# jsh58/Genrich

Hardware: AMD Instinct MI355X
Metric: genome bases p-scored/sec, hg38 50M frags (higher is better)
Workload: dtype int32 pileup (1/120 units) + f64 p-values; 1 GPU; hg38 25 contigs (3088286401 bp), 50000000 paired fragments x 1 replicate(s), treatment only, -p 0.01 (BASELINE.json configs[1]); parallelism=chromosome-sharded x1, collectives=none, rccl_nranks=0, intervals=83948696, tables_written_in_step=none: the sweep walks the loose (end, V) slots, p = table p(V)

## Files before the change

### genrich_amd/csrc/gx_host_ctx.h

```cpp
#pragma once
#include <hip/hip_runtime.h>
#include <rocprim/device/device_radix_sort.hpp>

#include <algorithm>
#include <cmath>
#include <cstdio>
#include <cstdlib>
#include <cstring>
#include <atomic>
#include <chrono>
#include <string>
#include <vector>
#include <unistd.h>

#include "gx_merge.h"
#include "gx_rccl.h"
#include "gx_sort.h"
#include "gx_tile_fast.h"
#include "gx_sbtile.h"
#include "gx_dups.h"
#include "gx_bhx.h"
#include "gx_saturate.h"
#include "gx_count.h"
#include "gx_regions.h"
#include "gx_coverage.h"
#include "gx_profile.h"
#include "gx_gram.h"
#include "gx_fingerprint.h"
#include "gx_rank.h"

using namespace gx;

namespace {

struct DevBuf {
  void* p = nullptr;
  size_t cap = 0;
  DevBuf() = default;
  DevBuf(const DevBuf&) = delete;
  DevBuf& operator=(const DevBuf&) = delete;
  DevBuf(DevBuf&& o) noexcept : p(o.p), cap(o.cap), own(o.own) { o.p = nullptr; o.cap = 0; o.own = true; }
  DevBuf& operator=(DevBuf&& o) noexcept {
    if (this != &o) { release(); p = o.p; cap = o.cap; own = o.own; o.p = nullptr; o.cap = 0; o.own = true; }
    return *this;
  }
  ~DevBuf() { release(); }
  void release() {
    if (p && own) (void)hipFree(p);
    p = nullptr;
    cap = 0;
    own = true;
  }
  void view(void* ptr, size_t bytes) {
    release();
    p = ptr;
    cap = bytes;
    own = false;
  }
  hipError_t ensure(size_t bytes) {
    if (bytes <= cap) return hipSuccess;
    release();
    size_t want = bytes + bytes / 8 + 256;
    hipError_t e = hipMalloc(&p, want);
    if (e == hipSuccess) cap = want;
    return e;
  }
  template <typename T> T* as() const { return reinterpret_cast<T*>(p); }
  bool own = true;
};

struct HostMail {
  Scalars scal;
  long long acc[2];
  uint64_t peakBP, genome;
  u32 nF, nIv, status, R, nPeaks, nMerged, D, n, hot, bhOvf;
  long long coll[4];
  u32 counts[64];
  u32 closeState;
  u32 statusKeep;
  u32 seq;
};

struct PinnedBuf {
  void* p = nullptr;
  void* dp = nullptr;
  size_t cap = 0;
  PinnedBuf() = default;
  PinnedBuf(const PinnedBuf&) = delete;
  PinnedBuf& operator=(const PinnedBuf&) = delete;
  ~PinnedBuf() { if (p) (void)hipHostFree(p); }
  hipError_t ensure(size_t bytes) {
    if (bytes <= cap) return hipSuccess;
    if (p) (void)hipHostFree(p);
    p = nullptr;
    cap = 0;
    size_t want = bytes + bytes / 4 + 4096;
    hipError_t e = hipHostMalloc(&p, want, hipHostMallocMapped | hipHostMallocCoherent);
    if (e == hipSuccess) {
      cap = want;
      e = hipHostGetDevicePointer(&dp, p, 0);
    }
    return e;
  }
};

struct Pileup {
  DevBuf ivEnd, ivV, tileIvOff, chromIvOff;
  u32 nIv = 0;
  bool packed = false;
  DevBuf looseEnd, looseV, meta;
  bool inLoose = false;
};

struct PArray {
  DevBuf end, p, expt, ctrl, chromOff, tileOff, q, dPresent;
  u32 n = 0;
  bool loose = false;
  bool looseSweep = false;
  DevBuf chromLooseOff;
  size_t looseStride = 0;
  bool pilesPending = false;
  bool pairPending = false;
  bool mergedP = false;
  DevBuf keptV, keptMeta;
  bool keptLoose = false;
  bool latePending = false, lateLoose = false;
  bool qLazy = false;
  bool hasPiles = false;
  bool pilesDropped = false;
  float ctrlConst = 0.0f;
  bool ctrlIsConst = false;
  std::vector<uint8_t> present;
};

struct Phase {
  std::string name;
  hipEvent_t a, b;
};

struct Knobs {
  int debug = 0;
  int debugRetry = 0;
  int noSpin = 0;
  int forceRec64 = 0;
  int forceSlowFrag = 0;
  int noFused = 0;
  int noLoose = 0;
  int noPairs = 0;
  int noFracPairs = 0;
  int noBedFused = 0;
  int bhVariant = -1;
  int mergeWg = 0;
  int noQLoose = 0;
  int noLateLoose = 0;
  int noLazyQ = 0;
  int noPackHist = 0;
  int noMergeP = 0;
  int forceHalfBins = 0;
  int noHalfBins = 0;
  int fracHalfBins = 0;
  int noEarlyColl = 0;
  int regWindows = 0;
  int noDenseBh = 0;
  int qtMulti = 0;
  int forceColl = 0;
  int sbShift = -1;
  long long runCapMin = 0;
  int bhCapLog = 0;
  int ptJmax = 0;
  int sbtTr = 0;
  int sbtGrid = 0;
  int s2Grid = 0;
  int fpAgg = 0;
  int rankCapLog = 0;
  int rankLookup = 0;
  int roctx = 0;
  int fault = 0;
};
struct BuildPlan {
  int isCtrl = 0;
  bool reuseSort = false;
  u32 nEv = 0;
  bool unit32 = false;
  bool multiRank = false;
  bool earlyColl = false;
  bool fused = false;
  bool pairs = false;
  bool fracPairs = false;
  int sbS = 0;
  u32 nL1 = 0;
  u32 nCoarse = 0, jmaxC = 0, nWG1 = 0;
  u32 jmax = 0;
  u32 poolPages[3] = {0, 0, 0};
  bool wantEarly = false;
  bool wantLate = false;
  bool closeInScan = false;
  bool dense = false;
  bool denseSmall = false;
  bool fragFused = false;
  size_t looseCap = 0, ivCap = 0;
  u32 tChunks = 0;
  bool masks() const { return wantEarly || wantLate; }
};
struct KnobDef { const char* name; int Knobs::*i; long long Knobs::*ll; };
const KnobDef KNOBS[] = {
    {"GX_DEBUG", &Knobs::debug, nullptr}, {"GX_DEBUG_RETRY", &Knobs::debugRetry, nullptr}, {"GX_NO_SPIN", &Knobs::noSpin, nullptr},
    {"GX_FORCE_REC64", &Knobs::forceRec64, nullptr}, {"GX_FORCE_SLOWFRAG", &Knobs::forceSlowFrag, nullptr},
    {"GX_NO_FUSED", &Knobs::noFused, nullptr}, {"GX_NO_LOOSE", &Knobs::noLoose, nullptr}, {"GX_NO_PAIRS", &Knobs::noPairs, nullptr},
    {"GX_NO_FRAC_PAIRS", &Knobs::noFracPairs, nullptr}, {"GX_NO_BED_FUSED", &Knobs::noBedFused, nullptr}, {"GX_NO_MERGE_P", &Knobs::noMergeP, nullptr}, {"GX_NO_PACK_HIST", &Knobs::noPackHist, nullptr}, {"GX_NO_LAZY_Q", &Knobs::noLazyQ, nullptr}, {"GX_NO_LATE_LOOSE", &Knobs::noLateLoose, nullptr}, {"GX_NO_Q_LOOSE", &Knobs::noQLoose, nullptr}, {"GX_MERGE_WG", &Knobs::mergeWg, nullptr}, {"GX_BH_VARIANT", &Knobs::bhVariant, nullptr}, {"GX_FORCE_HALF_BINS", &Knobs::forceHalfBins, nullptr},
    {"GX_NO_HALF_BINS", &Knobs::noHalfBins, nullptr}, {"GX_FRAC_HALF_BINS", &Knobs::fracHalfBins, nullptr}, {"GX_NO_EARLY_COLL", &Knobs::noEarlyColl, nullptr},
    {"GX_NO_DENSE_BH", &Knobs::noDenseBh, nullptr}, {"GX_REG_WINDOWS", &Knobs::regWindows, nullptr}, {"GX_QT_MULTI", &Knobs::qtMulti, nullptr}, {"GX_FORCE_COLL", &Knobs::forceColl, nullptr},
    {"GX_SBSHIFT", &Knobs::sbShift, nullptr}, {"GX_RUN_CAP_MIN", nullptr, &Knobs::runCapMin}, {"GX_BH_CAPLOG", &Knobs::bhCapLog, nullptr},
    {"GX_PT_JMAX", &Knobs::ptJmax, nullptr}, {"GX_FAULT", &Knobs::fault, nullptr}, {"GX_SBT_TR", &Knobs::sbtTr, nullptr}, {"GX_SBT_GRID", &Knobs::sbtGrid, nullptr},
    {"GX_S2_GRID", &Knobs::s2Grid, nullptr},
    {"GX_FP_AGG", &Knobs::fpAgg, nullptr},
    {"GX_RANK_CAP_LOG", &Knobs::rankCapLog, nullptr},
    {"GX_RANK_LOOKUP", &Knobs::rankLookup, nullptr},
    {"GX_ROCTX", &Knobs::roctx, nullptr},
};
bool set_knob(Knobs& k, const char* name, const char* value) {
  for (const KnobDef& d : KNOBS)
    if (!strcmp(d.name, name)) {
      long long v = 1;
      if (value && *value) {
        char* end = nullptr;
        v = strtoll(value, &end, 10);
        if (end == value) v = 1;
      }
      if (d.i) k.*(d.i) = (int)v; else k.*(d.ll) = v;
      return true;
    }
  return false;
}

}

struct gx_ctx {
  gx_params par{};
  Knobs knob;
  int device = 0;
  hipStream_t stream = nullptr;
  bool keepPiles = true;
  int maskIdx = -1;
  u32 maskN = 0;
  size_t maskStride = 0;
  hipStream_t side = nullptr;
  hipEvent_t sideEv = nullptr;
  std::string err;
  std::vector<uint32_t> len;
  std::vector<uint8_t> skip, save, owned;
  std::vector<std::vector<uint32_t>> bed;
  std::vector<DChrom> hChrom;
  u32 nChrom = 0, nTiles = 0;
  int sbShift = 0;
  u32 nSB = 0;
  DevBuf dChrom, dTileChrom, dBedTileOff, dBedEdge, dTileSave0;
  bool hasBed = false;
  bool bedGiven = false;
  size_t nBedEdges = 0;
  int phase = 0;
  int sample = 0;
  struct Seg { const gx_event* p; size_t n; hipEvent_t ready; bool packed = false; };
  std::vector<DevBuf> unpackBufs;
  size_t unpackUsed = 0;
  std::vector<Seg> segs;
  std::vector<DevBuf> evChunks;
  size_t evChunkIdx = 0, evChunkFill = 0;
  PinnedBuf stage[2];
  hipEvent_t stageFree[2] = {nullptr, nullptr};
  int stageNext = 0;
  std::vector<hipEvent_t> evPool;
  size_t evPoolUsed = 0;
  DevBuf satBuf;
  struct Stream {
    DevBuf a, pool, pt, cursor, sbOff;
  };
  size_t b2LdsSet = 0;
  bool sbtLdsSet = false;
  bool sawFrac = false;
  bool fracHint = false;
  bool fusedOff = false;
  BuildPlan built;
  bool earlyOwed = false;
  bool earlyPending = false;
  int fusedBackoff[2] = {0, 0};
  bool looseSwept = false;
  bool pilesMade = false;
  int denseHistIdx = -1;
  bool denseHistUsed = false;
  bool mergePUsed = false;
  DevBuf lbSweep, lbSweep2;
  u32 sweepGen = 0;
  FragSelect closeSel{};
  u32 closeSeq = 0;
  bool beginPending = false;
  u64 beginGenome = 0;
  bool fellBack = false;
  bool ptGrew = false;
  bool packedUsed = false;
  bool looseOk = false;
  bool riskNearThr = false;
  size_t looseStride = 0;
  DevBuf tileSlot, chromW0, chromLooseOff, looseCtl;
  u32 ptJmax = 16;
  DevBuf lbIv;
  Stream str[3];
  DevBuf tileCnt[3], tileOff[3];
  DevBuf looseC, looseC2, pairLogE, pairCtab, pairP2d, fragSum, tileDeep, fragList, zeroArena, endAtLen, binNet, curC, ptC, poolC, auxC, nWide, wideList, heavyList;
  size_t arenaBytes = 0;
  DevBuf tileMeta, tileWsum, tileCarry, lb, misc, dScal, dStatus, looseEnd, looseV, tileIvCount, tileLastEnd, tilePrevEnd;
  Pileup expt, ctrl;
  Scalars hScal{};
  std::vector<PArray> reps;
  int finalIdx = -1;
  DevBuf pvLut, dRisk, dDeep;
  PinnedBuf riskHost;
  bool pairTabsReady = false;
  DevBuf bhKeys, bhLens, bhOutKeys, bhOutSlot, bhSortKeys, bhSortSlot, bhQ, bhKQ, bhRaw, bhDl, bhTmp, bhRecs;
  PinnedBuf hostRecs;
  bool satDone = false;
  long long satDropped = 0;
  bool qLooseBad = false;
  bool qLooseUsed = false;
  DevBuf qLut;
  bool lateLooseUsed = false;
  bool lazyQUsed = false;
  bool bhLive = false;
  u32 bhLiveCap = 0;
  int bhLiveIdx = -1;
  bool bhDirty = false;
  u32 bhCapLog = 22;
  DevBuf swStart, swEnd, swMask, cand, valid, peaks, headPos, candHdr, longList;
  PinnedBuf hPeaks;
  size_t nHostPeaks = 0;
  u32* nIvTarget = nullptr;
  PinnedBuf mailBuf;
  HostMail* mail = nullptr;
  uint64_t genomeLenUsed = 0, peakBP = 0;
  int rank = 0, world = 1;
  gx_allreduce_i64_fn allreduce = nullptr;
  void* user = nullptr;
  ncclComm_t comm = nullptr;
  bool forceColl = false;
  DevBuf bigBins;
  DevBuf dColl, dCounts, dGather, bhDense, bhxSmall, bhxRecv, bhxKeys, bhxLens, bhxQ, bhxOut, bhxAns;
  bool rangeBhUsed = false;
  bool denseBhUsed = false;
  int phaseLevel = 0;
  std::string phaseFilter = "tile";
  u32 mailSeq = 0;
  u32 statusSeen = 1;
  u64 runCap = 0, runSeen = 0;
  bool phaseOpen = false;
  bool roctxOpen = false;
  int numCU = 0, resTile = 0, resTileHalf = 0, resTileFast = 0, resSweep = 0;
  int resSortA = 0, resSortB = 0;
  std::vector<DevBuf> pool;
  struct KeptSample {
    int rep = 0;
    bool ctrl = false;
    std::vector<Seg> segs;
    std::vector<uint8_t> save;
    std::vector<DevBuf> chunks, unpacks;
    DevBuf sat;
  };
  bool countOn = false;
  bool peaksReady = false;
// ... 293 lines not shown
```

### genrich_amd/csrc/gx_host_sweep.h

```cpp
#pragma once
namespace {

struct SweepSrc {
  const u32* end = nullptr;
  const float* p = nullptr;
  const float* q = nullptr;
  const u64* kq = nullptr;
  u32 kqMask = 0;
  const int* V = nullptr;
  const float* qLut = nullptr;
  bool haveMasks = false, hasSkip = true;
  const u32* chromOff = nullptr;
  u32 nChrom = 0, nWords = 0;
  size_t mStride = 0;
};

int run_sweep(gx_ctx* ctx, const SweepSrc& S, u32* nPeaksOut) {
  hipStream_t s = ctx->stream;
  u32* misc = ctx->misc.as<u32>();
  HostMail* dm = static_cast<HostMail*>(ctx->mailBuf.dp);
  const u32 nWords = S.nWords, nChrom = S.nChrom;
  const u32 wChunks = (nWords + SW_CHUNK - 1) / SW_CHUNK;
  SweepMasks SM{ctx->swMask.as<u64>(), ctx->swMask.as<u64>() + S.mStride, ctx->swMask.as<u64>() + 2 * S.mStride, nWords};
  if (S.V) SM = SweepMasks{ctx->swMask.as<u64>(), nullptr, ctx->swMask.as<u64>() + S.mStride, nWords};
  u32 R = 0, nPeaks = 0;
  ctx->peakBP = 0;
  ctx->nHostPeaks = 0;
  if (nWords) {
    if (!S.V) hipLaunchKernelGGL(k_brk_mask, dim3((nChrom + 255) / 256), dim3(256), 0, s, S.chromOff, nChrom, SM.brk);
    if (!S.haveMasks)
      hipLaunchKernelGGL(k_sig_mask, dim3(std::max(1u, std::min((nWords + 15) / 16, 4096u))), dim3(256), 0, s, S.p, S.q,
                         misc + M_NIV, ctx->par.thr, SM);
    {
      const size_t need = (size_t)2 * (wChunks + 8) * 8;
      if (ctx->lbSweep.cap < need) {
        HIPCHECK(ctx->lbSweep.ensure(need));
        HIPCHECK(hipMemsetAsync(ctx->lbSweep.p, 0, ctx->lbSweep.cap, s));
      }
    }
    for (int attempt = 0;; attempt++) {
      const u64 capMin = ctx->knob.runCapMin > 0 ? (u64)ctx->knob.runCapMin : (u64)1 << 16;
      const u64 guess = ctx->knob.runCapMin > 0 ? capMin : std::max<u64>(capMin, (u64)nWords / 4);
      const u32 cap = std::min<u64>(std::max<u64>(ctx->runCap, std::max<u64>(guess, 1)), (u64)nWords * 64);
      HIPCHECK(ctx->swStart.ensure((size_t)cap * 4 + 16));
      HIPCHECK(ctx->swEnd.ensure((size_t)cap * 4 + 16));
      HIPCHECK(ctx->headPos.ensure((size_t)cap * 4 + 16));
      HIPCHECK(ctx->cand.ensure((size_t)cap * sizeof(gx_peak)));
      HIPCHECK(ctx->valid.ensure((size_t)cap * 4 + 16));
      HIPCHECK(ctx->hPeaks.ensure((size_t)cap * sizeof(gx_peak) + 16));
      HIPCHECK(ctx->candHdr.ensure((size_t)cap * sizeof(uint4)));
      HIPCHECK(ctx->longList.ensure((size_t)cap * 4 + 16));
      const u32 rChunks = (cap + RC_CHUNK - 1) / RC_CHUNK;
      {
        const size_t need = (size_t)2 * (rChunks + 8) * 8;
        if (ctx->lbSweep2.cap < need) {
          HIPCHECK(ctx->lbSweep2.ensure(need));
          HIPCHECK(hipMemsetAsync(ctx->lbSweep2.p, 0, ctx->lbSweep2.cap, s));
        }
      }
      if (++ctx->sweepGen >= (1u << 24)) {
        ctx->sweepGen = 1;
        HIPCHECK(hipMemsetAsync(ctx->lbSweep.p, 0, ctx->lbSweep.cap, s));
        HIPCHECK(hipMemsetAsync(ctx->lbSweep2.p, 0, ctx->lbSweep2.cap, s));
      }
      const u32 gen = ctx->sweepGen;
      u64* lbS = ctx->lbSweep.as<u64>();
      u64* lbE = lbS + wChunks + 8;
      u64* lbC = ctx->lbSweep2.as<u64>();
      u64* lbP = lbC + rChunks + 8;
      u32* runStart = ctx->swStart.as<u32>();
      u32* runEnd = ctx->swEnd.as<u32>();
      const u64* skipM = S.hasSkip ? SM.skip : (const u64*)nullptr;
      const u32 gridP = (u32)std::max(1, ctx->resSweep);
      hipLaunchKernelGGL(k_runs, dim3(std::min<u32>(wChunks, gridP)), dim3(SW_NT), 0, s, SM, lbS, lbE, gen, runStart, runEnd, cap,
                         misc + M_SWCOUNT, &dm->R, misc + M_TICKET3, reinterpret_cast<u64*>(misc + M_PEAKBP), ctx->dStatus.as<u32>());
      hipLaunchKernelGGL(k_cands, dim3(std::min<u32>(rChunks, gridP)), dim3(SW_NT), 0, s, SM, skipM, S.end, runStart, runEnd,
                         misc + M_SWCOUNT, ctx->par.max_gap, S.chromOff, nChrom, lbC, gen, ctx->headPos.as<u32>(), misc + M_NHEADS,
                         ctx->dStatus.as<u32>());
      hipLaunchKernelGGL(k_cand_hdr, dim3(std::max(1u, std::min((cap + 255) / 256, 4096u))), dim3(256), 0, s, SM, S.end, runStart,
                         runEnd, misc + M_SWCOUNT, ctx->headPos.as<u32>(), misc + M_NHEADS, ctx->candHdr.as<uint4>(),
                         ctx->longList.as<u32>(), misc + M_TICKET3);
      if (S.kq)
        hipLaunchKernelGGL(k_q_fill_cands, dim3(std::max(1u, std::min((cap + 3) / 4, 32768u))), dim3(256), 0, s,
                           ctx->candHdr.as<uint4>(), misc + M_NHEADS, S.p, S.kq, S.kqMask, const_cast<float*>(S.q), ctx->dStatus.as<u32>());
      {
        const dim3 grid(std::max(1u, std::min((cap + 15) / 16, 16384u)));
        const dim3 gridW(std::max(1u, std::min((cap + 3) / 4, (u32)(8 * ctx->numCU))));
#define GX_LAUNCH_PEAKS(Q, V, NSHORT, QPTR)                                                                               \
  hipLaunchKernelGGL((k_peak_both<Q, V>), dim3((NSHORT) + gridW.x), dim3(256), 0, s, (u32)(NSHORT), ctx->candHdr.as<uint4>(), \
                     S.end, S.p, QPTR, S.chromOff, nChrom, misc + M_NHEADS, ctx->longList.as<u32>(), misc + M_TICKET3,       \
                     ctx->par.thr, ctx->par.min_auc, ctx->par.min_len, ctx->cand.as<gx_peak>(), ctx->valid.as<u32>())
        if (S.V && S.qLut) {
          const u32 nShortV = std::min<u32>(grid.x, (u32)(8 * ctx->numCU));
          hipLaunchKernelGGL((k_peak_both<false, true, true>), dim3(nShortV + gridW.x), dim3(256), 0, s, nShortV, ctx->candHdr.as<uint4>(),
                             S.end, S.p, reinterpret_cast<const float*>(S.V), S.chromOff, nChrom, misc + M_NHEADS, ctx->longList.as<u32>(),
                             misc + M_TICKET3, ctx->par.thr, ctx->par.min_auc, ctx->par.min_len, ctx->cand.as<gx_peak>(),
                             ctx->valid.as<u32>(), S.qLut);
        } else if (S.V) {
          const u32 nShortV = std::min<u32>(grid.x, (u32)(8 * ctx->numCU));
          GX_LAUNCH_PEAKS(false, true, nShortV, reinterpret_cast<const float*>(S.V));
        } else if (S.q)
          GX_LAUNCH_PEAKS(true, false, grid.x, S.q);
        else
          GX_LAUNCH_PEAKS(false, false, grid.x, S.q);
#undef GX_LAUNCH_PEAKS
      }
      hipLaunchKernelGGL(k_peaks, dim3(std::min<u32>(rChunks, gridP)), dim3(SW_NT), 0, s, ctx->cand.as<gx_peak>(), ctx->valid.as<u32>(),
                         misc + M_NHEADS, lbP, gen, static_cast<gx_peak*>(ctx->hPeaks.dp), misc + M_NPEAKS, &dm->nPeaks,
                         ctx->dStatus.as<u32>(), reinterpret_cast<u64*>(misc + M_PEAKBP));
      if (int rc__ = dbg_sync(ctx, "sweep kernels")) return rc__;
      if (int rc__ = mail_sync(ctx, nullptr, nullptr, nullptr, nullptr, nullptr, reinterpret_cast<const u64*>(misc + M_PEAKBP)))
        return rc__;
      R = ctx->mail->R;
      ctx->runSeen = R;
      if (R <= cap) break;
      if (attempt >= 2) {
        ctx->err = "peak sweep: run count changed between attempts";
        return GX_ERR_DEVICE;
      }
      ctx->runCap = (u64)R + R / 4 + 1024;
    }
    ctx->runCap = std::max<u64>(ctx->runCap, (u64)R + R / 4 + 1024);
  } else {
    if (int rc__ = mail_sync(ctx, nullptr, nullptr, nullptr, nullptr, nullptr)) return rc__;
  }
  if (R) nPeaks = ctx->mail->nPeaks;
  ctx->nHostPeaks = nPeaks;
  ctx->peakBP = R ? ctx->mail->peakBP : 0;
  *nPeaksOut = nPeaks;
  return status_to_rc(ctx, ctx->mail->status);
}

}
```

### genrich_amd/csrc/gx_stats.h

```cpp
#pragma once
#include "gx_kernels.h"

namespace gx {


__device__ __forceinline__ float pval_of_v(int v, float lambda, double ml, double sl, float* valOut, bool* neg, bool* risky) {
  float val = getval(v, neg);
  *valOut = val;
  if (lambda == 0.0f) return val == 0.0f ? 0.0f : FLT_MAX;
  return val == 0.0f ? 0.0f : pval_given(val, ml, sl, risky);
}

__device__ __forceinline__ void deep_risky_body(PackIn in, const FragFix* __restrict__ ff, const u32* __restrict__ list,
                                                const Scalars* __restrict__ sc, RiskBuf* __restrict__ risk, u32 block, u32 nBlocks);

__device__ __forceinline__ void lut_entry(u32 v, float lambda, double ml, double sl, float* __restrict__ lutP,
                                          RiskBuf* __restrict__ risk, LooseCtl* __restrict__ ctl, float thr, u32* red, u32 tid,
                                          u32 wg) {
  float val;
  bool ng, risky = false;
  const float p = pval_of_v((int)v, lambda, ml, sl, &val, &ng, &risky);
  lutP[v] = p;
  if (v % GX_UNIT == 0) lutP[PV_LUT + v / GX_UNIT] = p;
  if (risky) risk_add(risk, RK_LUT, v, 0, 0, 0.0);
// ... 996 lines not shown
constexpr int SW_NT = 256;
constexpr int SW_ITEMS = 8;
constexpr int SW_CHUNK = SW_NT * SW_ITEMS;
constexpr int RC_CHUNK = SW_NT;

__global__ void k_set_misc(u32* __restrict__ misc, u32 nivWord, u32 genomeWord, u64 genome, u32 n) {
  misc[nivWord] = n;
  *reinterpret_cast<u64*>(misc + genomeWord) = genome;
}

struct SweepMasks {
  u64* sig;
  u64* skip;
  u64* brk;
  u32 nWords;
};

__global__ void k_brk_mask(const u32* __restrict__ chromOff, u32 nChrom, u64* __restrict__ brk) {
  for (u32 c = blockIdx.x * blockDim.x + threadIdx.x; c < nChrom; c += gridDim.x * blockDim.x) {
    u32 a = chromOff[c], b = chromOff[c + 1];
    if (b > a) atomicOr(&brk[a >> 6], 1ull << (a & 63));
  }
}

__global__ __launch_bounds__(256) void k_sig_mask(const float* __restrict__ p, const float* __restrict__ q,
                                                  const u32* __restrict__ nPtr, float thr, SweepMasks M) {
  const u32 n = *nPtr;
  const float* pq = q ? q : p;
  const u32 nw = (n + 63) >> 6;
  for (u32 w0 = (blockIdx.x * 4 + (threadIdx.x >> 6)) * 4; w0 < nw; w0 += gridDim.x * 16) {
    float v[4];
#pragma unroll
    for (int k = 0; k < 4; k++) {
      const u32 i = ((w0 + k) << 6) + lane_id();
      v[k] = i < n ? pq[i] : 0.0f;
    }
#pragma unroll
    for (int k = 0; k < 4; k++) {
      const u64 sg = __ballot(v[k] > thr);
      const u64 sk = __ballot(v[k] == GX_SKIPF);
      if (lane_id() == 0 && w0 + k < nw) {
        M.sig[w0 + k] = sg;
        M.skip[w0 + k] = sk;
      }
    }
  }
}

__device__ __forceinline__ void run_bits(const SweepMasks& M, u32 w, u64* starts, u64* ends) {
  const u64 sg = M.sig[w], bk = M.brk[w];
  const u64 prevBit = w ? M.sig[w - 1] >> 63 : 0ull;
  const u64 nextBit = w + 1 < M.nWords ? M.sig[w + 1] & 1ull : 0ull;
  const u64 nextBrk = w + 1 < M.nWords ? M.brk[w + 1] & 1ull : 0ull;
  *starts = sg & (~((sg << 1) | prevBit) | bk);
  *ends = sg & (~((sg >> 1) | (nextBit << 63)) | ((bk >> 1) | (nextBrk << 63)));
}

__device__ __forceinline__ bool any_bit(const u64* __restrict__ mask, u32 lo, u32 hi) {
  if (lo >= hi) return false;
  u32 w0 = lo >> 6, w1 = (hi - 1) >> 6;
  for (u32 w = w0; w <= w1; w++) {
    u64 m = mask[w];
    if (w == w0) m &= ~0ull << (lo & 63);
    if (w == w1 && ((hi & 63) != 0)) m &= (1ull << (hi & 63)) - 1;
    if (m) return true;
  }
  return false;
}

__device__ __forceinline__ bool run_is_head(const SweepMasks& M, const u64* __restrict__ skipMask, const u32* __restrict__ end,
                                            const u32* __restrict__ runStart, const u32* __restrict__ runEnd, u32 r,
                                            int maxGap, const u32* __restrict__ chromOff, u32 nChrom) {
  if (r == 0) return true;
  const u32 a = runEnd[r - 1], s = runStart[r];
  if ((M.brk[s >> 6] >> (s & 63)) & 1ull) return true;
  ChromCursor cur;
  cur.seek(chromOff, nChrom, a);
  if (s >= cur.hi) return true;
  const long long gap = (long long)end[s - 1] - (long long)end[a];
  if (gap != 0 && gap > (long long)maxGap) return true;
  if (skipMask && any_bit(skipMask, a + 1, s)) return true;
  return false;
}

#ifndef GX_PK_SHORT
#define GX_PK_SHORT 1024
#endif
constexpr u32 PK_SHORT = GX_PK_SHORT;
#ifndef GX_PK_LOADS
#define GX_PK_LOADS 8
#endif
constexpr int PK_LOADS = GX_PK_LOADS;

__global__ __launch_bounds__(256) void k_cand_hdr(SweepMasks M, const u32* __restrict__ end,
                                                  const u32* __restrict__ runStart, const u32* __restrict__ runEnd,
                                                  const u32* __restrict__ nRuns, const u32* __restrict__ candRun,
                                                  const u32* __restrict__ nCands, uint4* __restrict__ hdr,
                                                  u32* __restrict__ longList, u32* __restrict__ nLong) {
  const u32 R = *nRuns, C = *nCands;
  for (u32 c = blockIdx.x * 256 + threadIdx.x; c < C; c += gridDim.x * 256) {
    const u32 rFirst = candRun[c], rLast = (c + 1 < C ? candRun[c + 1] : R) - 1;
    const u32 i0 = runStart[rFirst], i1 = runEnd[rLast];
    const bool atChromStart = (M.brk[i0 >> 6] >> (i0 & 63)) & 1ull;
    hdr[c] = make_uint4(i0, i1, atChromStart ? 0u : end[i0 - 1], end[i1]);
    if (i1 - i0 >= PK_SHORT) longList[atomicAdd(nLong, 1u)] = c;
  }
}

__device__ __forceinline__ void peak_finish(u32 c, const uint4 h, float auc, u32 summitPos, float sp, float sq,
                                            float minAUC, int minLen, const u32* __restrict__ chromOff, u32 nChrom,
                                            gx_peak* __restrict__ cand, u32* __restrict__ valid) {
  const u32 peakStart = h.z, peakEnd = h.w;
  const bool ok = auc >= minAUC && (long long)peakEnd - (long long)peakStart >= (long long)minLen;
  valid[c] = ok;
  if (ok) {
    ChromCursor cur;
    cur.seek(chromOff, nChrom, h.x);
    gx_peak pk;
    pk.chrom = cur.c;
    pk.start = peakStart;
    pk.end = peakEnd;
    pk.summit = summitPos;
    pk.auc = auc;
    pk.p = sp;
    pk.q = sq;
    cand[c] = pk;
  }
}

struct PeakAcc {
  float auc = 0.0f, summitVal = -1.0f, sp = -1.0f, sq = -1.0f;
  u32 summitPos = 0, summitLen = 0, s = 0, origin = 0;
  __device__ __forceinline__ void step(u32 e, float pv, float qv, bool useQ, float thr) {
    const float pq = useQ ? qv : pv;
    if (pq > thr) {
      auc += (float)(e - s) * (pq - thr);
      const u32 len = e - s;
      if (pq > summitVal) {
        summitVal = pq;
        sp = pv;
        sq = qv;
        summitPos = (u32)(((u64)e + s) / 2 - origin);
        summitLen = len;
      } else if (pq == summitVal && len > summitLen) {
        summitPos = (u32)(((u64)e + s) / 2 - origin);
        summitLen = len;
      }
    }
    s = e;
  }
};

template <int K> __device__ __forceinline__ float row_lane(float v) {
  return __int_as_float(__builtin_amdgcn_update_dpp(0, __float_as_int(v), 0x150 + K, 0xf, 0xf, false));
}
template <int K> struct RowSeqSum {
  static __device__ __forceinline__ float run(float acc, float v) { return RowSeqSum<K - 1>::run(acc, v) + row_lane<K>(v); }
};
template <> struct RowSeqSum<-1> { static __device__ __forceinline__ float run(float acc, float) { return acc; } };
__device__ __forceinline__ float row_max_f(float v) {
  v = fmaxf(v, __int_as_float(__builtin_amdgcn_update_dpp(0, __float_as_int(v), 0x128, 0xf, 0xf, false)));
  v = fmaxf(v, __int_as_float(__builtin_amdgcn_update_dpp(0, __float_as_int(v), 0x124, 0xf, 0xf, false)));
  v = fmaxf(v, __int_as_float(__builtin_amdgcn_update_dpp(0, __float_as_int(v), 0x122, 0xf, 0xf, false)));
  v = fmaxf(v, __int_as_float(__builtin_amdgcn_update_dpp(0, __float_as_int(v), 0x121, 0xf, 0xf, false)));
  return v;
}
__device__ __forceinline__ u32 row_max_u(u32 v) {
  v = max(v, (u32)__builtin_amdgcn_update_dpp(0, (int)v, 0x128, 0xf, 0xf, false));
  v = max(v, (u32)__builtin_amdgcn_update_dpp(0, (int)v, 0x124, 0xf, 0xf, false));
  v = max(v, (u32)__builtin_amdgcn_update_dpp(0, (int)v, 0x122, 0xf, 0xf, false));
  v = max(v, (u32)__builtin_amdgcn_update_dpp(0, (int)v, 0x121, 0xf, 0xf, false));
  return v;
}

constexpr int PK_AHEAD = 4;
#ifndef GX_PK_AHEAD_V
#define GX_PK_AHEAD_V 4
#endif
__device__ __forceinline__ void load_whole_lut(float* __restrict__ hot, const float* __restrict__ lut) {
  for (u32 i = threadIdx.x; i < PV_WHOLE; i += blockDim.x) hot[i] = lut[PV_LUT + i];
  __syncthreads();
}
__device__ __forceinline__ float p_from_v(const float* __restrict__ hot, const float* __restrict__ lut, const int* __restrict__ V, u32 i) {
  const u32 v = (u32)V[i];
  const u32 c = __umulhi(v, 0x88888889u) >> 6;
  if (v != c * (u32)GX_UNIT) return lut[v < PV_LUT ? v : 0u];
  return hot[c < PV_WHOLE ? c : 0u];
}
__device__ __forceinline__ float q_from_v(const float* __restrict__ hotq, const int* __restrict__ V, u32 i) {
  const u32 c = __umulhi((u32)V[i], 0x88888889u) >> 6;
  return hotq[c < PV_WHOLE ? c : 0u];
}
template <bool USEQ, bool PV, bool PVQ = false>
__device__ __forceinline__ void peak_short_body(const u32 blk, const u32 nBlk, const float* __restrict__ hot, const float* __restrict__ hotq,
                                                const uint4* __restrict__ hdr, const u32* __restrict__ end,
                                                const float* __restrict__ p, const float* __restrict__ q,
                                                const u32* __restrict__ chromOff, u32 nChrom,
                                                const u32* __restrict__ nCands, float thr, float minAUC, int minLen,
                                                gx_peak* __restrict__ cand, u32* __restrict__ valid) {
  constexpr int AH = PV ? GX_PK_AHEAD_V : PK_AHEAD;
  const u32 C = *nCands;
  const int lane = lane_id(), rowBase = lane & 48, rl = lane & 15;
  const u32 rowId = (blk * 4 + (threadIdx.x >> 6)) * 4 + (u32)(lane >> 4);
  for (u32 c0 = 0; c0 < C; c0 += nBlk * 16) {
    const u32 c = c0 + rowId;
    uint4 h = make_uint4(1u, 0u, 0u, 0u);
    if (c < C) h = hdr[c];
    const u32 i0 = h.x, i1 = h.y, peakStart = h.z;
    const bool mine = c < C && i1 - i0 < PK_SHORT;
    const u32 n = mine ? i1 - i0 + 1 : 0u;
    u32 steps = (n + 15) >> 4;
    steps = max(steps, (u32)__shfl_xor((int)steps, 16, 64));
    steps = max(steps, (u32)__shfl_xor((int)steps, 32, 64));
    float auc = 0.0f, summitVal = -1.0f, sp = -1.0f, sq = -1.0f;
    u32 summitPos = 0, summitLen = 0;
    for (u32 st0 = 0; st0 < steps; st0 += AH) {
      u32 e[AH], sPrev[AH];
      float pv[AH], qv[AH];
      bool in[AH];
#pragma unroll
      for (int a = 0; a < AH; a++) {
        const u32 i = i0 + (st0 + a) * 16 + rl;
        in[a] = mine && i <= i1;
        e[a] = 0; sPrev[a] = 0; pv[a] = 0.0f; qv[a] = GX_SKIPF;
        if (in[a]) {
          e[a] = end[i];
          sPrev[a] = i == i0 ? peakStart : end[i - 1];
          if (PV) pv[a] = p_from_v(hot, p, reinterpret_cast<const int*>(q), i);
          else pv[a] = p[i];
          if (USEQ) qv[a] = q[i];
          if (PVQ) qv[a] = q_from_v(hotq, reinterpret_cast<const int*>(q), i);
        }
      }
#pragma unroll
      for (int a = 0; a < AH; a++) {
        if (st0 + a >= steps) break;
        float pq = USEQ || PVQ ? qv[a] : pv[a];
        const bool sg = in[a] && pq > thr;
        float term = 0.0f;
        if (sg) term = (float)(e[a] - sPrev[a]) * (pq - thr);
        else pq = -2.0f;
        const u64 wSg = __ballot(sg);
        if (wSg) {
          auc = RowSeqSum<15>::run(auc, term);
          const float mx = row_max_f(pq);
          const bool atMax = sg && pq == mx;
          const u32 len = atMax ? e[a] - sPrev[a] : 0u;
          const u32 ml = row_max_u(len);
          const bool rowSg = ((u32)(wSg >> rowBase) & 0xFFFFu) != 0;
          const bool better = rowSg && mx > summitVal, longer = rowSg && mx == summitVal && ml > summitLen;
          if (__ballot(better || longer)) {
            const u32 rowMax = (u32)(__ballot(atMax) >> rowBase) & 0xFFFFu;
            const u32 rowLen = (u32)(__ballot(atMax && len == ml) >> rowBase) & 0xFFFFu;
            const int firstMax = rowBase + (rowMax ? __builtin_ctz(rowMax) : 0);
            const int firstLen = rowBase + (rowLen ? __builtin_ctz(rowLen) : 0);
            const u32 myPos = (u32)(((u64)e[a] + sPrev[a]) / 2 - peakStart);
            const u32 cPos = (u32)__shfl((int)myPos, firstLen, 64);
            const float spN = __shfl(pv[a], firstMax, 64), sqN = __shfl(qv[a], firstMax, 64);
            if (better) {
              summitVal = mx;
              sp = spN;
              sq = sqN;
              summitPos = cPos;
              summitLen = ml;
            } else if (longer) {
              summitPos = cPos;
              summitLen = ml;
            }
          }
        }
      }
    }
    if (mine && rl == 0) peak_finish(c, h, auc, summitPos, sp, sq, minAUC, minLen, chromOff, nChrom, cand, valid);
  }
}

template <bool PV, bool PVQ = false>
__device__ __forceinline__ void peak_walk_body(const u32 blk, const u32 nBlk, const float* __restrict__ hot, const float* __restrict__ hotq,
                                               const uint4* __restrict__ hdr, const u32* __restrict__ end,
                                               const float* __restrict__ p, const float* __restrict__ qIn,
                                               const u32* __restrict__ chromOff, u32 nChrom,
                                               const u32* __restrict__ longList, const u32* __restrict__ nLong,
                                               float thr, float minAUC, int minLen,
                                               gx_peak* __restrict__ cand, u32* __restrict__ valid) {
  constexpr int AH = PV ? GX_PK_AHEAD_V : PK_AHEAD;
  const float* __restrict__ q = PV ? nullptr : qIn;
  const u32 L = *nLong;
  const u32 wavesPerGrid = nBlk * 4;
  const int lane = lane_id();
  auto rdf = [](float v, int l) -> float { return __int_as_float(__builtin_amdgcn_readlane(__float_as_int(v), l)); };
  for (u32 li = blk * 4 + (threadIdx.x >> 6); li < L; li += wavesPerGrid) {
    const u32 c = longList[li];
    const uint4 h = hdr[c];
    const u32 i0 = h.x, i1 = h.y, peakStart = h.z;
    float auc = 0.0f, summitVal = -1.0f, sp = -1.0f, sq = -1.0f;
    u32 summitPos = 0, summitLen = 0;
    for (u32 base = i0; base <= i1; base += 64 * AH) {
      u32 e[AH], sPrev[AH];
      float pv[AH], qv[AH];
      bool in[AH];
#pragma unroll
      for (int a = 0; a < AH; a++) {
        const u32 i = base + a * 64 + lane;
        in[a] = i <= i1;
        e[a] = 0; sPrev[a] = 0; pv[a] = 0.0f; qv[a] = GX_SKIPF;
        if (in[a]) {
          e[a] = end[i];
          sPrev[a] = i == i0 ? peakStart : end[i - 1];
          if (PV) pv[a] = p_from_v(hot, p, reinterpret_cast<const int*>(qIn), i);
          else pv[a] = p[i];
          if (q) qv[a] = q[i];
          if (PVQ) qv[a] = q_from_v(hotq, reinterpret_cast<const int*>(qIn), i);
        }
      }
#pragma unroll
      for (int a = 0; a < AH; a++) {
        if (base + a * 64 > i1) break;
        float pq = q || PVQ ? qv[a] : pv[a];
        const bool sg = in[a] && pq > thr;
        float term = 0.0f;
        if (sg) term = (float)(e[a] - sPrev[a]) * (pq - thr);
        else pq = -2.0f;
        if (__ballot(sg)) {
          float acc = RowSeqSum<15>::run(auc, term);
          acc = RowSeqSum<15>::run(rdf(acc, 0), term);
          acc = RowSeqSum<15>::run(rdf(acc, 16), term);
          acc = RowSeqSum<15>::run(rdf(acc, 32), term);
          auc = rdf(acc, 48);
          float mx = row_max_f(pq);
          mx = fmaxf(fmaxf(rdf(mx, 0), rdf(mx, 16)), fmaxf(rdf(mx, 32), rdf(mx, 48)));
          const bool atMax = sg && pq == mx;
          const u32 len = atMax ? e[a] - sPrev[a] : 0u;
          u32 ml = row_max_u(len);
          ml = max(max((u32)__builtin_amdgcn_readlane((int)ml, 0), (u32)__builtin_amdgcn_readlane((int)ml, 16)),
                   max((u32)__builtin_amdgcn_readlane((int)ml, 32), (u32)__builtin_amdgcn_readlane((int)ml, 48)));
          if (mx > summitVal || (mx == summitVal && ml > summitLen)) {
            const int firstMax = __builtin_ctzll(__ballot(atMax));
            const int firstLen = __builtin_ctzll(__ballot(atMax && len == ml));
            const u32 myPos = (u32)(((u64)e[a] + sPrev[a]) / 2 - peakStart);
            const u32 cPos = (u32)__builtin_amdgcn_readlane((int)myPos, firstLen);
            if (mx > summitVal) {
              summitVal = mx;
              sp = rdf(pv[a], firstMax);
              sq = rdf(qv[a], firstMax);
            }
            summitPos = cPos;
            summitLen = ml;
          }
        }
      }
    }
    if (lane == 0) peak_finish(c, h, auc, summitPos, sp, sq, minAUC, minLen, chromOff, nChrom, cand, valid);
  }
}

template <bool USEQ, bool PV, bool PVQ = false>
__global__ __launch_bounds__(256) void k_peak_both(u32 nShort, const uint4* __restrict__ hdr, const u32* __restrict__ end,
                                                   const float* __restrict__ p, const float* __restrict__ q,
                                                   const u32* __restrict__ chromOff, u32 nChrom,
                                                   const u32* __restrict__ nCands, const u32* __restrict__ longList,
                                                   const u32* __restrict__ nLong, float thr, float minAUC, int minLen,
                                                   gx_peak* __restrict__ cand, u32* __restrict__ valid,
                                                   const float* __restrict__ qLut = nullptr) {
  static_assert(!PVQ || (PV && !USEQ), "q by pileup rides the sweep on the loose slots");
  __shared__ float hot[PV ? PV_WHOLE : 1];
  __shared__ float hotq[PVQ ? PV_WHOLE : 1];
  const u32 nWalk = gridDim.x - nShort;
#ifndef GX_PK_NO_EARLY_EXIT
  if (blockIdx.x < nWalk && blockIdx.x * 4 >= *nLong) return;
#endif
  if (PVQ)
    for (u32 i = threadIdx.x; i < PV_WHOLE; i += blockDim.x) hotq[i] = qLut[i];
  if (PV) load_whole_lut(hot, p);
  if (blockIdx.x >= nWalk)
    peak_short_body<USEQ, PV, PVQ>(blockIdx.x - nWalk, nShort, hot, hotq, hdr, end, p, q, chromOff, nChrom, nCands, thr, minAUC, minLen, cand, valid);
  else
    peak_walk_body<PV, PVQ>(blockIdx.x, nWalk, hot, hotq, hdr, end, p, q, chromOff, nChrom, longList, nLong, thr, minAUC, minLen, cand, valid);
}

constexpr int LBG_SHIFT = 38;
__device__ __forceinline__ u64 lookback_gen(u64* lb, u32 id, u64 aggregate, u32 gen, u32* st) {
  const u64 tag = (u64)(gen & 0xFFFFFFu) << LBG_SHIFT, vmask = (1ull << LBG_SHIFT) - 1;
  u64 excl = 0;
  if (id > 0) {
    if (lane_id() == 0)
      __hip_atomic_store(&lb[id], LB_AGG | tag | (aggregate & vmask), __ATOMIC_RELAXED, __HIP_MEMORY_SCOPE_AGENT);
    int look = (int)id - 1;
    u32 spins = 0;
    bool done = false;
    while (!done) {
      const int idx = look - lane_id();
      u64 v = idx >= 0 ? __hip_atomic_load(&lb[idx], __ATOMIC_RELAXED, __HIP_MEMORY_SCOPE_AGENT) : (LB_INC | tag);
      if (((v >> LBG_SHIFT) & 0xFFFFFFu) != (gen & 0xFFFFFFu)) v = 0;
      const u64 flag = v >> 62;
      const u64 invalidMask = __ballot(flag == 0), incMask = __ballot(flag == 2);
      const int firstInvalid = invalidMask ? __builtin_ctzll(invalidMask) : 64;
      const int firstInc = incMask ? __builtin_ctzll(incMask) : 64;
      if (firstInc < firstInvalid) {
        excl += wave_sum(lane_id() <= firstInc ? (v & vmask) : 0ull);
        done = true;
      } else if (firstInvalid > 0) {
        excl += wave_sum(lane_id() < firstInvalid ? (v & vmask) : 0ull);
        look -= firstInvalid;
      } else {
        __builtin_amdgcn_s_sleep(1);
        ++spins;
        bool abort_ = spins > LB_SPIN_LIMIT;
        if (!abort_ && (spins & 1023u) == 0)
          abort_ = (__hip_atomic_load(st, __ATOMIC_RELAXED, __HIP_MEMORY_SCOPE_AGENT) & ST_LOOKBACK) != 0;
        if (abort_) {
          if (lane_id() == 0) atomicOr(st, ST_LOOKBACK);
          done = true;
        }
      }
    }
  }
  excl &= vmask;
  if (lane_id() == 0)
    __hip_atomic_store(&lb[id], LB_INC | tag | ((excl + aggregate) & vmask), __ATOMIC_RELAXED, __HIP_MEMORY_SCOPE_AGENT);
  return excl;
}

__global__ __launch_bounds__(SW_NT) void k_runs(SweepMasks M, u64* __restrict__ lbS, u64* __restrict__ lbE, u32 gen,
                                                u32* __restrict__ runStart, u32* __restrict__ runEnd, u32 cap,
                                                u32* __restrict__ nRuns , u32* __restrict__ nRunsHost ,
                                                u32* __restrict__ zeroMe, u64* __restrict__ zeroBp, u32* __restrict__ st) {
  __shared__ u32 scratch[8];
  __shared__ u64 s_base[2];
  const u32 nChunks = (M.nWords + SW_CHUNK - 1) / SW_CHUNK;
  for (u32 id = blockIdx.x; id < nChunks; id += gridDim.x) {
    const u32 w0 = id * SW_CHUNK + threadIdx.x * SW_ITEMS;
    u64 stb[SW_ITEMS], enb[SW_ITEMS];
    u32 a = 0, b = 0;
#pragma unroll
    for (int k = 0; k < SW_ITEMS; k++) {
      stb[k] = 0;
      enb[k] = 0;
      if (w0 + k < M.nWords) run_bits(M, w0 + k, &stb[k], &enb[k]);
      a += __popcll(stb[k]);
      b += __popcll(enb[k]);
    }
    u32 totA;
    u32 oa = block_excl_scan<u32, SW_NT>(a, scratch, &totA);
    (void)b;
    if (threadIdx.x < 64) {
      const u64 ea = lookback_gen(lbS, id, totA, gen, st);
      if (threadIdx.x == 0) {
        s_base[0] = ea;
        if (id == nChunks - 1) {
          const u32 total = (u32)ea + totA;
          *nRuns = total > cap ? cap : total;
          *nRunsHost = total;
          *zeroMe = 0;
          *zeroBp = 0;
        }
      }
    }
    __syncthreads();
    oa += (u32)s_base[0];
    u32 ob = oa;
    if (w0 < M.nWords) {
      const u64 sig0 = M.sig[w0];
      ob -= (u32)(sig0 & ~stb[0] & 1ull);
    }
#ifdef GX_RUNS_TWO_SCANS
    {
      u32 totB;
      ob = block_excl_scan<u32, SW_NT>(b, scratch, &totB);
      __shared__ u64 s_b;
      if (threadIdx.x < 64) {
        const u64 eb = lookback_gen(lbE, id, totB, gen, st);
        if (threadIdx.x == 0) s_b = eb;
      }
      __syncthreads();
      ob += (u32)s_b;
    }
#endif
#pragma unroll
    for (int k = 0; k < SW_ITEMS; k++) {
      u64 x = stb[k];
      while (x) {
        const int bit = __builtin_ctzll(x);
        x &= x - 1;
        if (oa < cap) runStart[oa] = ((w0 + k) << 6) + bit;
        oa++;
      }
      x = enb[k];
      while (x) {
        const int bit = __builtin_ctzll(x);
        x &= x - 1;
        if (ob < cap) runEnd[ob] = ((w0 + k) << 6) + bit;
        ob++;
      }
    }
    __syncthreads();
  }
}

__global__ __launch_bounds__(SW_NT) void k_cands(SweepMasks M, const u64* __restrict__ skipMask, const u32* __restrict__ end,
                                                 const u32* __restrict__ runStart, const u32* __restrict__ runEnd,
                                                 const u32* __restrict__ nRuns, int maxGap, const u32* __restrict__ chromOff,
                                                 u32 nChrom, u64* __restrict__ lb, u32 gen, u32* __restrict__ candRun,
                                                 u32* __restrict__ nCands, u32* __restrict__ st) {
  __shared__ u32 scratch[8];
// ... 75 lines not shown
```

Before: 2777 Gbases/s.

## Defer summit reduction to per-lane accumulators and derive previous end via DPP

Each lane now keeps a running summit (best p, longest run, position), and the cross-lane max/min reduction happens once per peak instead of on every step. The previous-interval end comes from the neighbouring lane through a DPP shift plus a carried value, which removes the second load of end[i-1]. The RowSeqSum DPP bound_ctrl flag is flipped, and an optional GX_SW_GRID knob is added to cap the sweep grid. This cuts per-step wave reductions and ballots in the peak kernels. The risk is subtle tie-break or carry errors, for example in the row-mode carry and the bound_ctrl change altering the AUC sums.

```diff
diff --git a/genrich_amd/csrc/gx_host_ctx.h b/genrich_amd/csrc/gx_host_ctx.h
--- a/genrich_amd/csrc/gx_host_ctx.h
+++ b/genrich_amd/csrc/gx_host_ctx.h
@@ -171,6 +171,7 @@
   int sbtTr = 0;
   int sbtGrid = 0;
   int s2Grid = 0;
+  int swGrid = 0;
   int fpAgg = 0;
   int rankCapLog = 0;
   int rankLookup = 0;
@@ -212,7 +213,7 @@
     {"GX_NO_DENSE_BH", &Knobs::noDenseBh, nullptr}, {"GX_REG_WINDOWS", &Knobs::regWindows, nullptr}, {"GX_QT_MULTI", &Knobs::qtMulti, nullptr}, {"GX_FORCE_COLL", &Knobs::forceColl, nullptr},
     {"GX_SBSHIFT", &Knobs::sbShift, nullptr}, {"GX_RUN_CAP_MIN", nullptr, &Knobs::runCapMin}, {"GX_BH_CAPLOG", &Knobs::bhCapLog, nullptr},
     {"GX_PT_JMAX", &Knobs::ptJmax, nullptr}, {"GX_FAULT", &Knobs::fault, nullptr}, {"GX_SBT_TR", &Knobs::sbtTr, nullptr}, {"GX_SBT_GRID", &Knobs::sbtGrid, nullptr},
-    {"GX_S2_GRID", &Knobs::s2Grid, nullptr},
+    {"GX_S2_GRID", &Knobs::s2Grid, nullptr}, {"GX_SW_GRID", &Knobs::swGrid, nullptr},
     {"GX_FP_AGG", &Knobs::fpAgg, nullptr},
     {"GX_RANK_CAP_LOG", &Knobs::rankCapLog, nullptr},
     {"GX_RANK_LOOKUP", &Knobs::rankLookup, nullptr},
diff --git a/genrich_amd/csrc/gx_host_sweep.h b/genrich_amd/csrc/gx_host_sweep.h
--- a/genrich_amd/csrc/gx_host_sweep.h
+++ b/genrich_amd/csrc/gx_host_sweep.h
@@ -71,7 +71,8 @@
       u32* runStart = ctx->swStart.as<u32>();
       u32* runEnd = ctx->swEnd.as<u32>();
       const u64* skipM = S.hasSkip ? SM.skip : (const u64*)nullptr;
-      const u32 gridP = (u32)std::max(1, ctx->resSweep);
+      u32 gridP = (u32)std::max(1, ctx->resSweep);
+      if (ctx->knob.swGrid > 0) gridP = std::min<u32>(gridP, (u32)ctx->knob.swGrid);
       hipLaunchKernelGGL(k_runs, dim3(std::min<u32>(wChunks, gridP)), dim3(SW_NT), 0, s, SM, lbS, lbE, gen, runStart, runEnd, cap,
                          misc + M_SWCOUNT, &dm->R, misc + M_TICKET3, reinterpret_cast<u64*>(misc + M_PEAKBP), ctx->dStatus.as<u32>());
       hipLaunchKernelGGL(k_cands, dim3(std::min<u32>(rChunks, gridP)), dim3(SW_NT), 0, s, SM, skipM, S.end, runStart, runEnd,
diff --git a/genrich_amd/csrc/gx_stats.h b/genrich_amd/csrc/gx_stats.h
--- a/genrich_amd/csrc/gx_stats.h
+++ b/genrich_amd/csrc/gx_stats.h
@@ -1172,7 +1172,7 @@
 };
 
 template <int K> __device__ __forceinline__ float row_lane(float v) {
-  return __int_as_float(__builtin_amdgcn_update_dpp(0, __float_as_int(v), 0x150 + K, 0xf, 0xf, false));
+  return __int_as_float(__builtin_amdgcn_update_dpp(0, __float_as_int(v), 0x150 + K, 0xf, 0xf, true));
 }
 template <int K> struct RowSeqSum {
   static __device__ __forceinline__ float run(float acc, float v) { return RowSeqSum<K - 1>::run(acc, v) + row_lane<K>(v); }
@@ -1192,6 +1192,67 @@
   v = max(v, (u32)__builtin_amdgcn_update_dpp(0, (int)v, 0x121, 0xf, 0xf, false));
   return v;
 }
+__device__ __forceinline__ u32 row_min_u(u32 v) {
+  v = min(v, (u32)__builtin_amdgcn_update_dpp(0, (int)v, 0x128, 0xf, 0xf, false));
+  v = min(v, (u32)__builtin_amdgcn_update_dpp(0, (int)v, 0x124, 0xf, 0xf, false));
+  v = min(v, (u32)__builtin_amdgcn_update_dpp(0, (int)v, 0x122, 0xf, 0xf, false));
+  v = min(v, (u32)__builtin_amdgcn_update_dpp(0, (int)v, 0x121, 0xf, 0xf, false));
+  return v;
+}
+template <bool WAVE> __device__ __forceinline__ float all_max_f(float v) {
+  v = row_max_f(v);
+  if (WAVE) {
+    auto rd = [](float x, int l) -> float { return __int_as_float(__builtin_amdgcn_readlane(__float_as_int(x), l)); };
+    v = fmaxf(fmaxf(rd(v, 0), rd(v, 16)), fmaxf(rd(v, 32), rd(v, 48)));
+  }
+  return v;
+}
+template <bool WAVE> __device__ __forceinline__ u32 all_max_u(u32 v) {
+  v = row_max_u(v);
+  if (WAVE)
+    v = max(max((u32)__builtin_amdgcn_readlane((int)v, 0), (u32)__builtin_amdgcn_readlane((int)v, 16)),
+            max((u32)__builtin_amdgcn_readlane((int)v, 32), (u32)__builtin_amdgcn_readlane((int)v, 48)));
+  return v;
+}
+template <bool WAVE> __device__ __forceinline__ u32 all_min_u(u32 v) {
+  v = row_min_u(v);
+  if (WAVE)
+    v = min(min((u32)__builtin_amdgcn_readlane((int)v, 0), (u32)__builtin_amdgcn_readlane((int)v, 16)),
+            min((u32)__builtin_amdgcn_readlane((int)v, 32), (u32)__builtin_amdgcn_readlane((int)v, 48)));
+  return v;
+}
+template <bool WAVE> __device__ __forceinline__ u32 prev_lane_u(u32 e, u32 first) {
+  return (u32)__builtin_amdgcn_update_dpp((int)first, (int)e, WAVE ? 0x138 : 0x111, 0xf, 0xf, false);
+}
+
+struct SummitAcc {
+  float best = -1.0f, sp = -1.0f, sq = -1.0f;
+  u32 iMax = ~0u;
+  u32 len = 0, end = 0, iLen = ~0u;
+  __device__ __forceinline__ void step(u32 i, u32 e, u32 l, float pq, float pv, float qv) {
+    const bool better = pq > best, moved = better | ((pq == best) & (l > len));
+    best = better ? pq : best;
+    sp = better ? pv : sp;
+    sq = better ? qv : sq;
+    iMax = better ? i : iMax;
+    len = moved ? l : len;
+    end = moved ? e : end;
+    iLen = moved ? i : iLen;
+  }
+  template <bool WAVE> __device__ __forceinline__ void join(u32 origin, float* spOut, float* sqOut, u32* posOut) const {
+    const float mx = all_max_f<WAVE>(best);
+    const bool atMax = best == mx;
+    const u32 first = all_min_u<WAVE>(atMax ? iMax : ~0u);
+    const bool winP = atMax && iMax == first;
+    *spOut = __uint_as_float(all_max_u<WAVE>(winP ? __float_as_uint(sp) : 0u));
+    *sqOut = __uint_as_float(all_max_u<WAVE>(winP ? __float_as_uint(sq) : 0u));
+    const u32 ml = all_max_u<WAVE>(atMax ? len : 0u);
+    const bool longest = atMax && len == ml;
+    const u32 firstLen = all_min_u<WAVE>(longest ? iLen : ~0u);
+    const u32 pos = iLen != ~0u ? (u32)(((u64)end + (end - len)) / 2 - origin) : 0u;
+    *posOut = all_max_u<WAVE>(longest && iLen == firstLen ? pos : 0u);
+  }
+};
 
 constexpr int PK_AHEAD = 4;
 #ifndef GX_PK_AHEAD_V
@@ -1232,20 +1293,21 @@
     u32 steps = (n + 15) >> 4;
     steps = max(steps, (u32)__shfl_xor((int)steps, 16, 64));
     steps = max(steps, (u32)__shfl_xor((int)steps, 32, 64));
-    float auc = 0.0f, summitVal = -1.0f, sp = -1.0f, sq = -1.0f;
-    u32 summitPos = 0, summitLen = 0;
+    float auc = 0.0f;
+    SummitAcc top;
+    u32 carry = peakStart;
     for (u32 st0 = 0; st0 < steps; st0 += AH) {
-      u32 e[AH], sPrev[AH];
+      u32 e[AH], idx[AH];
       float pv[AH], qv[AH];
       bool in[AH];
 #pragma unroll
       for (int a = 0; a < AH; a++) {
         const u32 i = i0 + (st0 + a) * 16 + rl;
+        idx[a] = i;
         in[a] = mine && i <= i1;
-        e[a] = 0; sPrev[a] = 0; pv[a] = 0.0f; qv[a] = GX_SKIPF;
+        e[a] = 0; pv[a] = 0.0f; qv[a] = GX_SKIPF;
         if (in[a]) {
           e[a] = end[i];
-          sPrev[a] = i == i0 ? peakStart : end[i - 1];
           if (PV) pv[a] = p_from_v(hot, p, reinterpret_cast<const int*>(q), i);
           else pv[a] = p[i];
           if (USEQ) qv[a] = q[i];
@@ -1255,42 +1317,22 @@
 #pragma unroll
       for (int a = 0; a < AH; a++) {
         if (st0 + a >= steps) break;
+        const u32 len = e[a] - prev_lane_u<false>(e[a], carry);
+        carry = (u32)__builtin_amdgcn_update_dpp(0, (int)e[a], 0x15F, 0xf, 0xf, true);
         float pq = USEQ || PVQ ? qv[a] : pv[a];
         const bool sg = in[a] && pq > thr;
         float term = 0.0f;
-        if (sg) term = (float)(e[a] - sPrev[a]) * (pq - thr);
+        if (sg) term = (float)len * (pq - thr);
         else pq = -2.0f;
-        const u64 wSg = __ballot(sg);
-        if (wSg) {
+        if (__ballot(sg)) {
           auc = RowSeqSum<15>::run(auc, term);
-          const float mx = row_max_f(pq);
-          const bool atMax = sg && pq == mx;
-          const u32 len = atMax ? e[a] - sPrev[a] : 0u;
-          const u32 ml = row_max_u(len);
-          const bool rowSg = ((u32)(wSg >> rowBase) & 0xFFFFu) != 0;
-          const bool better = rowSg && mx > summitVal, longer = rowSg && mx == summitVal && ml > summitLen;
-          if (__ballot(better || longer)) {
-            const u32 rowMax = (u32)(__ballot(atMax) >> rowBase) & 0xFFFFu;
-            const u32 rowLen = (u32)(__ballot(atMax && len == ml) >> rowBase) & 0xFFFFu;
-            const int firstMax = rowBase + (rowMax ? __builtin_ctz(rowMax) : 0);
-            const int firstLen = rowBase + (rowLen ? __builtin_ctz(rowLen) : 0);
-            const u32 myPos = (u32)(((u64)e[a] + sPrev[a]) / 2 - peakStart);
-            const u32 cPos = (u32)__shfl((int)myPos, firstLen, 64);
-            const float spN = __shfl(pv[a], firstMax, 64), sqN = __shfl(qv[a], firstMax, 64);
-            if (better) {
-              summitVal = mx;
-              sp = spN;
-              sq = sqN;
-              summitPos = cPos;
-              summitLen = ml;
-            } else if (longer) {
-              summitPos = cPos;
-              summitLen = ml;
-            }
-          }
+          top.step(idx[a], e[a], len, pq, pv[a], qv[a]);
         }
       }
     }
+    float sp, sq;
+    u32 summitPos;
+    top.join<false>(peakStart, &sp, &sq, &summitPos);
     if (mine && rl == 0) peak_finish(c, h, auc, summitPos, sp, sq, minAUC, minLen, chromOff, nChrom, cand, valid);
   }
 }
@@ -1313,20 +1355,20 @@
     const u32 c = longList[li];
     const uint4 h = hdr[c];
     const u32 i0 = h.x, i1 = h.y, peakStart = h.z;
-    float auc = 0.0f, summitVal = -1.0f, sp = -1.0f, sq = -1.0f;
-    u32 summitPos = 0, summitLen = 0;
+    float auc = 0.0f;
+    SummitAcc top;
+    u32 carry = peakStart;
     for (u32 base = i0; base <= i1; base += 64 * AH) {
-      u32 e[AH], sPrev[AH];
+      u32 e[AH];
       float pv[AH], qv[AH];
       bool in[AH];
 #pragma unroll
       for (int a = 0; a < AH; a++) {
         const u32 i = base + a * 64 + lane;
         in[a] = i <= i1;
-        e[a] = 0; sPrev[a] = 0; pv[a] = 0.0f; qv[a] = GX_SKIPF;
+        e[a] = 0; pv[a] = 0.0f; qv[a] = GX_SKIPF;
         if (in[a]) {
           e[a] = end[i];
-          sPrev[a] = i == i0 ? peakStart : end[i - 1];
           if (PV) pv[a] = p_from_v(hot, p, reinterpret_cast<const int*>(qIn), i);
           else pv[a] = p[i];
           if (q) qv[a] = q[i];
@@ -1336,10 +1378,12 @@
 #pragma unroll
       for (int a = 0; a < AH; a++) {
         if (base + a * 64 > i1) break;
+        const u32 len = e[a] - prev_lane_u<true>(e[a], carry);
+        carry = (u32)__builtin_amdgcn_readlane((int)e[a], 63);
         float pq = q || PVQ ? qv[a] : pv[a];
         const bool sg = in[a] && pq > thr;
         float term = 0.0f;
-        if (sg) term = (float)(e[a] - sPrev[a]) * (pq - thr);
+        if (sg) term = (float)len * (pq - thr);
         else pq = -2.0f;
         if (__ballot(sg)) {
           float acc = RowSeqSum<15>::run(auc, term);
@@ -1347,29 +1391,13 @@
           acc = RowSeqSum<15>::run(rdf(acc, 16), term);
           acc = RowSeqSum<15>::run(rdf(acc, 32), term);
           auc = rdf(acc, 48);
-          float mx = row_max_f(pq);
-          mx = fmaxf(fmaxf(rdf(mx, 0), rdf(mx, 16)), fmaxf(rdf(mx, 32), rdf(mx, 48)));
-          const bool atMax = sg && pq == mx;
-          const u32 len = atMax ? e[a] - sPrev[a] : 0u;
-          u32 ml = row_max_u(len);
-          ml = max(max((u32)__builtin_amdgcn_readlane((int)ml, 0), (u32)__builtin_amdgcn_readlane((int)ml, 16)),
-                   max((u32)__builtin_amdgcn_readlane((int)ml, 32), (u32)__builtin_amdgcn_readlane((int)ml, 48)));
-          if (mx > summitVal || (mx == summitVal && ml > summitLen)) {
-            const int firstMax = __builtin_ctzll(__ballot(atMax));
-            const int firstLen = __builtin_ctzll(__ballot(atMax && len == ml));
-            const u32 myPos = (u32)(((u64)e[a] + sPrev[a]) / 2 - peakStart);
-            const u32 cPos = (u32)__builtin_amdgcn_readlane((int)myPos, firstLen);
-            if (mx > summitVal) {
-              summitVal = mx;
-              sp = rdf(pv[a], firstMax);
-              sq = rdf(qv[a], firstMax);
-            }
-            summitPos = cPos;
-            summitLen = ml;
-          }
+          top.step(base + a * 64 + lane, e[a], len, pq, pv[a], qv[a]);
         }
       }
     }
+    float sp, sq;
+    u32 summitPos;
+    top.join<true>(peakStart, &sp, &sq, &summitPos);
     if (lane == 0) peak_finish(c, h, auc, summitPos, sp, sq, minAUC, minLen, chromOff, nChrom, cand, valid);
   }
 }
```

New measurement: 2761 Gbases/s. No clear change (-0.6%).
